# qiangbo1222/HierDiff

Hardware: AMD Instinct MI355X
Metric: sampled molecules/sec (1000 diffusion steps, B=256, N=30) (higher is better)
Workload: dtype f32

## Files before the change

### hierdiff_amd/build.py

```python
from __future__ import annotations

import os
import shutil
import subprocess
import sys

PKG = os.path.dirname(os.path.abspath(__file__))
CSRC = os.path.join(PKG, "csrc")
LIBDIR = os.path.join(PKG, "lib")
LIB = os.path.join(LIBDIR, "libhierdiff_hip.so")
SOURCES = [os.path.join(CSRC, "hierdiff_hip.hip")]
DEPS = SOURCES + [os.path.join(CSRC, f) for f in sorted(os.listdir(CSRC)) if f.endswith(".hpp")] + [
    os.path.join(os.path.dirname(PKG), "include", "hierdiff_hip.h")]


def _hipcc() -> str:
    for cand in (os.environ.get("HIPCC"), shutil.which("hipcc"), "/opt/rocm/bin/hipcc"):
        if cand and os.path.exists(cand):
            return cand
    raise RuntimeError("hipcc not found (set HIPCC)")


def needs_build() -> bool:
    if not os.path.exists(LIB):
        return True
    t = os.path.getmtime(LIB)
    return any(os.path.getmtime(d) > t for d in DEPS)


RESOURCES = os.path.join(LIBDIR, "kernel_resources.json")
KERNEL_FLAGS = ["--offload-arch=gfx950", "-O3", "-fno-slp-vectorize", "-std=c++17"]


def _parse_resource_remarks(text: str) -> dict:
    import re
    out, cur = {}, None
    for line in text.splitlines():
        m = re.search(r"remark: Function Name: (\S+)", line)
        if m:
            cur = out.setdefault(m.group(1), {})
            continue
        m = re.search(r"remark:\s+([A-Za-z][A-Za-z /\[\]]*?)(?: \[[^\]]*\])?: (\S+) \[-Rpass", line)
        if m and cur is not None:
            key = m.group(1).strip()
            try:
                cur[key] = int(m.group(2))
            except ValueError:
                cur[key] = m.group(2)
    return out


def _production(name: str) -> bool:
    import re
    m = re.match(r"_Z6k_edgeILi\d+ELb[01]ELi[03]ELi(\d+)EE", name)
    if m:
        return m.group(1) == "0"
    return True


def audit(resources: dict) -> list:
    bad = []
    for name, r in resources.items():
        if not name.startswith("_Z") or not _production(name):
            continue
        if r.get("ScratchSize", 0) or r.get("VGPRs Spill", 0):
            bad.append(f"{name}: scratch {r.get('ScratchSize')} B/lane, VGPR spills {r.get('VGPRs Spill')}")
    return bad


LIB_DEBUG = os.path.join(LIBDIR, "libhierdiff_hip_dbg.so")


def build(force: bool = False, save_temps: bool = False, verbose: bool = True, debug_kernels: bool = False) -> str:
    if debug_kernels:
        return _build_debug(verbose)
    if not force and not needs_build() and os.path.exists(RESOURCES):
        return LIB
    os.makedirs(LIBDIR, exist_ok=True)
    cmd = [_hipcc()] + KERNEL_FLAGS + ["-fPIC", "-shared",
           "-Wall", "-Wno-unused-function", "-Wno-unused-value", "-Wno-unused-result",
           "-Rpass-analysis=kernel-resource-usage", "-o", LIB + ".tmp"] + SOURCES
    if save_temps:
        tmpdir = os.path.join(PKG, "build")
        os.makedirs(tmpdir, exist_ok=True)
        cmd += ["-save-temps=obj"]
    if verbose:
        print(" ".join(cmd), flush=True)
    proc = subprocess.run(cmd, cwd=CSRC, stderr=subprocess.PIPE, text=True)
    other = [ln for ln in proc.stderr.splitlines() if "-Rpass-analysis=kernel-resource-usage" not in ln
             and not ln.startswith("In file included from")]
    if other and (verbose or proc.returncode):
        print("\n".join(other), file=sys.stderr, flush=True)
    if proc.returncode:
        raise subprocess.CalledProcessError(proc.returncode, cmd)
    resources = _parse_resource_remarks(proc.stderr)
    import json
    with open(RESOURCES, "w") as fh:
        json.dump(resources, fh, indent=1, sort_keys=True)
    bad = audit(resources)
    if bad:
        raise RuntimeError("register spills in production kernels (unsafe next to inline-asm loads):\n  " + "\n  ".join(bad))
    os.replace(LIB + ".tmp", LIB)
    return LIB


def _build_debug(verbose: bool = True) -> str:
    os.makedirs(LIBDIR, exist_ok=True)
    cmd = [_hipcc(), "-DHD_DEBUG_KERNELS"] + KERNEL_FLAGS + ["-fPIC",
           "-shared", "-Wno-unused-function", "-Wno-unused-value", "-Wno-unused-result", "-o", LIB_DEBUG] + SOURCES
    if verbose:
        print(" ".join(cmd), flush=True)
    subprocess.run(cmd, cwd=CSRC, check=True)
    return LIB_DEBUG


if __name__ == "__main__":
    print(build(force="--force" in sys.argv, save_temps="--save-temps" in sys.argv,
                debug_kernels="--debug-kernels" in sys.argv))
```

### hierdiff_amd/csrc/hierdiff_hip.hip

```cpp
#include "../../include/hierdiff_hip.h"
#include "kernels.hpp"

#include <algorithm>
#include <array>
#include <cmath>
#include <cstdio>
#include <cstring>
#include <cstdlib>
#include <string>
#include <mutex>
#include <vector>


static thread_local std::string g_err;

static int fail(int code, const std::string& msg) {
    g_err = msg;
    return code;
}

#define HIP_TRY(expr)                                                                        \
    do {                                                                                     \
        hipError_t _e = (expr);                                                              \
        if (_e != hipSuccess)                                                                \
// ... 1232 lines not shown
        case 1024: run(std::integral_constant<int, 1024>{}); return true;
        case 1025: run(std::integral_constant<int, 1025>{}); return true;
        default: return false;
    }
}
#else
extern "C" int hd_debug_edge_trace(hd_handle*, long long*, int) { return 0; }
#endif

static bool edge_runs_split(const hd_handle* h, int n_tiles, int mode) {
    return n_tiles > 0 && n_tiles <= (mode == 0 ? h->split_max_tiles + h->split_max_tiles / 3 : h->split_max_tiles);
}
static bool edge_runs_mixed(const hd_handle* h, int n_tiles, int mode) {
    const int per_round = 4 * h->n_cu;
    const int left = n_tiles - (n_tiles / per_round) * per_round;
    const bool pays = left > 0 && left * 10 <= (mode == 0 ? 29 : 10) * h->n_cu;
    return n_tiles > per_round && n_tiles < h->mix_max_tiles && (pays || h->mix_rounds >= 0);
}

template <int H>
static int launch_edge_h(hd_handle* h, bool coord, const EdgeArgs& a, hipStream_t s, int mode_override = -1) {
    const int lds = edge_lds_bytes<H>();
    const int prec = mode_override >= 0 ? mode_override : h->edge_mode;
    const dim3 grid(a.n_wg), block(256);
    if constexpr (H >= 128) {
        if (a.dscal) {
            if (a.pre2) {
                if (coord) hipLaunchKernelGGL((k_edge<H, true, 3, HD_EDGE_SAVE | HD_EDGE_UNSCALED>), grid, block, lds, s, a);
                else hipLaunchKernelGGL((k_edge<H, false, 3, HD_EDGE_SAVE | HD_EDGE_UNSCALED>), grid, block, lds, s, a);
            } else {
                if (coord) hipLaunchKernelGGL((k_edge<H, true, 3, HD_EDGE_UNSCALED>), grid, block, lds, s, a);
                else hipLaunchKernelGGL((k_edge<H, false, 3, HD_EDGE_UNSCALED>), grid, block, lds, s, a);
            }
            return HD_OK;
        }
    }
    if (a.pre2) {
        if (coord) hipLaunchKernelGGL((k_edge<H, true, 0, HD_EDGE_SAVE>), grid, block, lds, s, a);
        else hipLaunchKernelGGL((k_edge<H, false, 0, HD_EDGE_SAVE>), grid, block, lds, s, a);
        return HD_OK;
    }
#ifdef HD_DEBUG_KERNELS
    if constexpr (H == 256) {
        if (h->ablate && !coord && (prec == 3 ? launch_edge_ablated<3>(h, a, s) : launch_edge_ablated<0>(h, a, s))) return HD_OK;
    }
#endif
    if constexpr (H >= 128) {
        const int mode = prec;
        if (edge_runs_split(h, a.n_tiles, mode)) {
            const dim3 sgrid(a.n_tiles);
            if (mode == 0) {
                if (coord) hipLaunchKernelGGL((k_edge_split<H, true, 0>), sgrid, block, 0, s, a);
                else hipLaunchKernelGGL((k_edge_split<H, false, 0>), sgrid, block, 0, s, a);
            } else {
                if (coord) hipLaunchKernelGGL((k_edge_split<H, true, 3>), sgrid, block, 0, s, a);
                else hipLaunchKernelGGL((k_edge_split<H, false, 3>), sgrid, block, 0, s, a);
            }
            return HD_OK;
        }
    }
    if constexpr (H >= 128) {
        const int mode = prec;
        const int per_round = 4 * h->n_cu;
        int R = a.n_tiles / per_round;
        if (edge_runs_mixed(h, a.n_tiles, mode)) {
            if (h->mix_rounds >= 0) R = std::min(R, h->mix_rounds);
            EdgeArgs m = a;
            m.n_wg = R * h->n_cu;
            const dim3 mgrid(m.n_wg + (a.n_tiles - 4 * m.n_wg));
            const int ldsm = std::max(edge_lds_bytes<H>(), edge_split_lds_bytes<H>());
            if (mode == 0) {
                if (coord) hipLaunchKernelGGL((k_edge_mixed<H, true, 0>), mgrid, block, ldsm, s, m);
                else hipLaunchKernelGGL((k_edge_mixed<H, false, 0>), mgrid, block, ldsm, s, m);
            } else {
                if (coord) hipLaunchKernelGGL((k_edge_mixed<H, true, 3>), mgrid, block, ldsm, s, m);
                else hipLaunchKernelGGL((k_edge_mixed<H, false, 3>), mgrid, block, ldsm, s, m);
            }
            return HD_OK;
        }
    }
    if (prec == 3) {
        if (coord) hipLaunchKernelGGL((k_edge<H, true, 3>), grid, block, lds, s, a);
        else hipLaunchKernelGGL((k_edge<H, false, 3>), grid, block, lds, s, a);
    } else {
        if (coord) hipLaunchKernelGGL((k_edge<H, true, 0>), grid, block, lds, s, a);
        else hipLaunchKernelGGL((k_edge<H, false, 0>), grid, block, lds, s, a);
    }
    return HD_OK;
}

template <int H>
static int prepare_edge_h() {
    const int lds = edge_lds_bytes<H>();
    HIP_TRY(hipFuncSetAttribute((const void*)k_edge<H, true, 0>, hipFuncAttributeMaxDynamicSharedMemorySize, lds));
    HIP_TRY(hipFuncSetAttribute((const void*)k_edge<H, false, 0>, hipFuncAttributeMaxDynamicSharedMemorySize, lds));
    HIP_TRY(hipFuncSetAttribute((const void*)k_edge<H, true, 3>, hipFuncAttributeMaxDynamicSharedMemorySize, lds));
    HIP_TRY(hipFuncSetAttribute((const void*)k_edge<H, false, 3>, hipFuncAttributeMaxDynamicSharedMemorySize, lds));
    HIP_TRY(hipFuncSetAttribute((const void*)k_edge<H, true, 0, HD_EDGE_SAVE>, hipFuncAttributeMaxDynamicSharedMemorySize, lds));
    HIP_TRY(hipFuncSetAttribute((const void*)k_edge<H, false, 0, HD_EDGE_SAVE>, hipFuncAttributeMaxDynamicSharedMemorySize, lds));
    if constexpr (H >= 128) {
        HIP_TRY(hipFuncSetAttribute((const void*)k_edge<H, true, 3, HD_EDGE_SAVE | HD_EDGE_UNSCALED>, hipFuncAttributeMaxDynamicSharedMemorySize, lds));
        HIP_TRY(hipFuncSetAttribute((const void*)k_edge<H, false, 3, HD_EDGE_SAVE | HD_EDGE_UNSCALED>, hipFuncAttributeMaxDynamicSharedMemorySize, lds));
        HIP_TRY(hipFuncSetAttribute((const void*)k_edge<H, true, 3, HD_EDGE_UNSCALED>, hipFuncAttributeMaxDynamicSharedMemorySize, lds));
        HIP_TRY(hipFuncSetAttribute((const void*)k_edge<H, false, 3, HD_EDGE_UNSCALED>, hipFuncAttributeMaxDynamicSharedMemorySize, lds));
        const int m0 = std::max(edge_lds_bytes<H>(), edge_split_lds_bytes<H>());
        HIP_TRY(hipFuncSetAttribute((const void*)k_edge_mixed<H, true, 0>, hipFuncAttributeMaxDynamicSharedMemorySize, m0));
        HIP_TRY(hipFuncSetAttribute((const void*)k_edge_mixed<H, false, 0>, hipFuncAttributeMaxDynamicSharedMemorySize, m0));
        HIP_TRY(hipFuncSetAttribute((const void*)k_edge_mixed<H, true, 3>, hipFuncAttributeMaxDynamicSharedMemorySize, m0));
        HIP_TRY(hipFuncSetAttribute((const void*)k_edge_mixed<H, false, 3>, hipFuncAttributeMaxDynamicSharedMemorySize, m0));
    }
    return HD_OK;
}

static int prepare_kernels(hd_handle* h) {
    switch (h->H) {
        case 32: HD_TRY(prepare_node_h<32>()); HD_TRY(prepare_edge_bwd_h<32>()); return prepare_edge_h<32>();
        case 64: HD_TRY(prepare_node_h<64>()); HD_TRY(prepare_edge_bwd_h<64>()); return prepare_edge_h<64>();
        case 128: HD_TRY(prepare_node_h<128>()); HD_TRY(prepare_node_split_h<128>()); HD_TRY(prepare_edge_bwd_h<128>()); return prepare_edge_h<128>();
        default: HD_TRY(prepare_node_h<256>()); HD_TRY(prepare_node_split_h<256>()); HD_TRY(prepare_edge_bwd_h<256>()); return prepare_edge_h<256>();
    }
}

static int edge(hd_handle* h, bool coord, const EdgeArgs& a, hipStream_t s, int mode_override = -1) {
    if (a.n_wg == 0) return HD_OK;
    ProfScope ps(h, s, 0);
    switch (h->H) {
        case 32: return launch_edge_h<32>(h, coord, a, s, mode_override);
        case 64: return launch_edge_h<64>(h, coord, a, s, mode_override);
        case 128: return launch_edge_h<128>(h, coord, a, s, mode_override);
        default: return launch_edge_h<256>(h, coord, a, s, mode_override);
    }
}

static int forward_impl(hd_handle* h, hd_topology* t, const float* xh, const float* tt, int t_numel,
                        const float* context, int mol_shape, float* out, hipStream_t s) {
    const hd_config& c = h->cfg;
    const int H = h->H, M = t->M;
    const float* W = h->dw;
    h->prof_now = h->prof != 0 && (h->prof_fwd++ % h->prof_stride) == 0;
    if (M == 0) HIP_TRY(hipMemsetAsync(h->d_nanflag, 0, sizeof(int), s));
    if (M > 0) {
        {
            ProfScope ps(h, s, 2);
            InitArgs a;
            a.xh = xh; a.t = tt; a.ctx = context; a.node_of = t->node_of; a.nmask = t->nmask;
            a.embT = W + h->embT; a.emb_b = W + h->emb_b; a.h = t->hbuf; a.x0 = t->x0; a.xcur = t->xcur;
            a.nanflag = h->d_nanflag;
            a.zero_max = (h->node_mode == 3 && M < h->node_split_max_rows && h->edge_mode == 3) ? t->abmax : nullptr;
            a.M = M; a.N = t->N; a.D = h->D; a.F = h->F; a.C = c.context_node_nf; a.H = H;
            a.t_stride = (t_numel == 1) ? 0 : 1; a.cond_time = c.condition_time;
            const long long total = (long long)M * (H / 4);
            hipLaunchKernelGGL(k_node_init, dim3((unsigned)((total + 255) / 256)), dim3(256), 0, s, a);
        }
        const float range = c.coords_range / (float)c.n_layers;
        const int S = c.inv_sublayers;
        const float* ab_cur = t->AB;
        auto node_args = [&]() {
            NodeArgs a;
            std::memset(&a, 0, sizeof(a));
            a.h_in = t->hbuf; a.h_out = t->hbuf; a.part = t->part; a.pstart = t->pstart; a.nmask = t->nmask;
            a.norm = agg_norm(c, t); a.M = M;
            return a;
        };
        auto set_ab = [&](NodeArgs& a, int q, const LayerW& nw, float* dst) {
            a.ABimg[q] = W + nw.ab_img; a.ABbias[q] = W + nw.ab_bias; a.ABout[q] = dst;
            a.abinv[q] = h->node_mode == 3 ? 1.0f / nw.abs_ : 1.0f;
            a.ABmax[q] = (h->edge_mode == 3 && h->node_mode != 0) ? (dst == t->AB ? t->abmax : t->abmax2) : nullptr;
        };
        const bool fused = h->node_mode != 0 || M >= h->fuse_min_rows;
        auto r16_args = [&]() {
            R16Args g;
            std::memset(&g, 0, sizeof(g));
            g.A = t->hbuf; g.lda = H; g.K1 = H; g.K = H; g.M = M; g.n_img = 1; g.nmask = t->nmask; g.norm = agg_norm(c, t);
            return g;
        };
        auto ab_r16 = [&](int nab, const LayerW* const* nxt, float* const* dst) {
            R16Args g = r16_args();
            g.Nc = 2 * H; g.ldc = 2 * H; g.n_img = nab;
            for (int q = 0; q < nab; ++q) { g.Bimg[q] = W + nxt[q]->ab_gimg; g.bias[q] = W + nxt[q]->ab_bias; g.C[q] = dst[q]; }
            gemm_r16(h, EPI_BIAS, false, g, s);
        };
        const bool nsplit = h->node_mode == 3 && M < h->node_split_max_rows;
// ... 1311 lines not shown
```

### hierdiff_amd/csrc/k_edge.hpp

```cpp
#pragma once
#include "common.hpp"


#ifndef HD_F32_SILU
#define HD_F32_SILU silu_fast
#define HD_F32_SILU_IS_FAST 1
#endif

struct EdgeArgs {
    const float* AB;
    const float* wrd;
    const float* W2img;
    const float* b2;
    const float* wa;
    const int* ei;
    const int* ej;
    const uint8_t* eseg;
    const int* seg_part;
    const int* tile_nseg;
    const float* xcur;
    const float* x0;
    float* part;
    float ba;
    const float* ba_ptr;
    float norm_constant;
    float coords_range;
    int attention, use_tanh;
    int n_tiles, n_wg;
    long long* trace;
    float w2s_inv;
    float wrmax, wdmax;
    const float* abmax;
    const float* dscal;
    float* pre2;
};

constexpr int HD_EDGE_SAVE = 256;
constexpr int HD_EDGE_UNSCALED = 512;
constexpr float HD_NEG_LOG2E = -1.4426950408889634f;


struct AbMaxArgs { const float* AB; float* out; int M, H; };
__global__ void __launch_bounds__(256) k_ab_rowmax(AbMaxArgs a) {
    const int row = blockIdx.x * 4 + (threadIdx.x >> 6), lane = threadIdx.x & 63;
    if (row >= a.M) return;
    const float* r = a.AB + (size_t)row * 2 * a.H;
    float ma = 0.f, mb = 0.f;
    for (int k = 4 * lane; k < a.H; k += 256) {
        const f32x4 va = *reinterpret_cast<const f32x4*>(r + k), vb = *reinterpret_cast<const f32x4*>(r + a.H + k);
#pragma unroll
        for (int j = 0; j < 4; ++j) { ma = fmaxf(ma, fabsf(va[j])); mb = fmaxf(mb, fabsf(vb[j])); }
    }
#pragma unroll
    for (int o = 32; o > 0; o >>= 1) { ma = fmaxf(ma, __shfl_xor(ma, o)); mb = fmaxf(mb, __shfl_xor(mb, o)); }
    if (lane == 0) { a.out[2 * (size_t)row] = ma; a.out[2 * (size_t)row + 1] = mb; }
}


template <typename V, unsigned O0, unsigned O1, unsigned O2, unsigned O3>
HD_DEVINL void lds_read4(V (&f)[4], unsigned addr) {
    asm volatile("ds_read_b128 %0, %4 offset:%5\n\t"
                 "ds_read_b128 %1, %4 offset:%6\n\t"
                 "ds_read_b128 %2, %4 offset:%7\n\t"
                 "ds_read_b128 %3, %4 offset:%8"
                 : "=&v"(f[0]), "=&v"(f[1]), "=&v"(f[2]), "=&v"(f[3])
                 : "v"(addr), "i"(O0), "i"(O1), "i"(O2), "i"(O3));
}
template <typename V, unsigned O>
HD_DEVINL void lds_read1(V& f, unsigned addr) {
    asm volatile("ds_read_b128 %0, %1 offset:%2" : "=&v"(f) : "v"(addr), "i"(O));
}
template <int N, typename V>
HD_DEVINL void lds_wait4(V (&f)[4]) {
    asm volatile("s_waitcnt lgkmcnt(%4)" : "+v"(f[0]), "+v"(f[1]), "+v"(f[2]), "+v"(f[3]) : "i"(N));
}

HD_DEVINL float xhalf_sum(float x) {
    float lo = x, hi = x;
    asm("s_nop 1\n\tv_permlane32_swap_b32 %0, %1\n\ts_nop 1" : "+v"(lo), "+v"(hi));
    return lo + hi;
}
HD_DEVINL void xhalf_sum4(float (&x)[4]) {
    float lo[4], hi[4];
#pragma unroll
    for (int k = 0; k < 4; ++k) { lo[k] = x[k]; hi[k] = x[k]; }
    asm("s_nop 1\n\t"
        "v_permlane32_swap_b32 %0, %4\n\tv_permlane32_swap_b32 %1, %5\n\t"
        "v_permlane32_swap_b32 %2, %6\n\tv_permlane32_swap_b32 %3, %7\n\t"
        "s_nop 1"
        : "+v"(lo[0]), "+v"(lo[1]), "+v"(lo[2]), "+v"(lo[3]), "+v"(hi[0]), "+v"(hi[1]), "+v"(hi[2]), "+v"(hi[3]));
#pragma unroll
    for (int k = 0; k < 4; ++k) x[k] = lo[k] + hi[k];
}

HD_DEVINL void vm_load2(f32x4& va, f32x4& vb, const float* pa, const float* pb) {
    asm volatile("global_load_dwordx4 %0, %2, off\n\t"
                 "global_load_dwordx4 %1, %3, off"
                 : "=&v"(va), "=&v"(vb) : "v"(pa), "v"(pb));
}
template <int OFF>
HD_DEVINL void vm_load2o(f32x4& va, f32x4& vb, const float* pa, const float* pb) {
    static_assert(OFF >= 0 && OFF < 4096, "immediate offset out of range");
    asm volatile("global_load_dwordx4 %0, %2, off offset:%4\n\t"
                 "global_load_dwordx4 %1, %3, off offset:%4"
                 : "=&v"(va), "=&v"(vb) : "v"(pa), "v"(pb), "i"(OFF));
}
HD_DEVINL void vm_glds2(const float* ga, const float* gb, unsigned lds_a, unsigned lds_b) {
    unsigned keep;
    asm volatile("s_mov_b32 %0, m0\n\t"
                 "s_mov_b32 m0, %3\n\ts_nop 0\n\tglobal_load_lds_dwordx4 %1, off\n\t"
                 "s_mov_b32 m0, %4\n\ts_nop 0\n\tglobal_load_lds_dwordx4 %2, off\n\t"
                 "s_mov_b32 m0, %0"
                 : "=&s"(keep) : "v"(ga), "v"(gb), "s"(lds_a), "s"(lds_b));
}
template <int N, unsigned OA, unsigned OB>
HD_DEVINL void lds_read2_after_vm(f32x4& qa, f32x4& qb, unsigned addr) {
    asm volatile("s_waitcnt vmcnt(%3)\n\t"
                 "ds_read_b128 %0, %2 offset:%4\n\t"
                 "ds_read_b128 %1, %2 offset:%5"
                 : "=&v"(qa), "=&v"(qb) : "v"(addr), "i"(N), "i"(OA), "i"(OB));
}
HD_DEVINL void lds_ready2(f32x4& qa, f32x4& qb) { asm volatile("s_waitcnt lgkmcnt(0)" : "+v"(qa), "+v"(qb)); }
// ... 28 lines not shown
    constexpr int GL_PER_WAVE = (ABL & 128) ? CHF / (4 * 256) / 4 : CHF / (4 * 256);
    constexpr int LEVEL = edge_peel_level(H, PREC, ABL);
    static_assert(LEVEL >= 0 && LEVEL <= 2, "peel level");
    constexpr bool HAS_PEN = LEVEL >= 2, HAS_LAST = LEVEL >= 1;
    float* wbuf = smem;
    float* scratch = smem + 2 * CHF + 2 * H;

    const int tid = threadIdx.x, lane = tid & 63;
    const int wave = __builtin_amdgcn_readfirstlane(tid >> 6);
    const int hh = lane >> 5, n = lane & 31;
    float* my_scr = scratch + wave * 136;
    uint32_t* seg_s = reinterpret_cast<uint32_t*>(my_scr + 128);

    int wt;
    {
        const int xcd = bid & 7, slot = bid >> 3;
        const int q = nwt >> 3, r = nwt & 7;
        const int start = xcd < r ? xcd * (q + 1) : r * (q + 1) + (xcd - r) * q;
        const int len = q + (xcd < r ? 1 : 0);
        if (slot >= len) return;
        wt = start + slot;
    }
    long long ts0 = 0, ts1 = 0, ts2 = 0, ts3 = 0, ts4 = 0, ts5 = 0;
    if constexpr (ABL & 16) ts0 = __builtin_readcyclecounter();

    for (int k = tid; k < 2 * H; k += 256) wrd_s[k] = a.wrd[k];
    for (int k = tid; k < H; k += 256) { wrd_s[2 * H + k] = a.b2[k]; wrd_s[3 * H + k] = a.wa[k]; }
    auto issue_chunk = [&](int c, int buf) {
        const float* src = a.W2img + (size_t)c * CHF + wave * (GL_PER_WAVE * 256) + lane * 4;
        float* dst = wbuf + buf * CHF + wave * (GL_PER_WAVE * 256);
        static_for<0, GL_PER_WAVE>([&](auto U) {
            constexpr int u = decltype(U)::value;
            glds16o<(u & 3) * 1024>(src + (u >> 2) * 1024, dst + (u >> 2) * 1024);
        });
    };
    issue_chunk(0, 0);

    const int tile = wt * 4 + wave;
    const bool tile_ok = tile < a.n_tiles;
    int ni = 0, nj = 0;
    uint32_t segb = 255;
    if (tile_ok) {
        const int e = tile * 32 + n;
        ni = a.ei[e]; nj = a.ej[e]; segb = a.eseg[e];
    }

    int gc = 0;
    f32x4 xi = *reinterpret_cast<const f32x4*>(a.xcur + (size_t)ni * 4);
    f32x4 xj = *reinterpret_cast<const f32x4*>(a.xcur + (size_t)nj * 4);
    f32x4 yi = *reinterpret_cast<const f32x4*>(a.x0 + (size_t)ni * 4);
    f32x4 yj = *reinterpret_cast<const f32x4*>(a.x0 + (size_t)nj * 4);
    const float dx = xi[0] - xj[0], dy = xi[1] - xj[1], dz = xi[2] - xj[2];
    const float radial = dx * dx + dy * dy + dz * dz;
    if constexpr (COORD) {
        if (hh == 0) {
            const float inv = ((segb != 255) ? 1.0f : 0.0f) / (sqrtf(radial + 1e-8f) + a.norm_constant);
            float* tr = my_scr + 32;
            tr[n * 3 + 0] = dx * inv; tr[n * 3 + 1] = dy * inv; tr[n * 3 + 2] = dz * inv;
        }
    }
    const float ex = yi[0] - yj[0], ey = yi[1] - yj[1], ez = yi[2] - yj[2];
    const float d0 = ex * ex + ey * ey + ez * ez;
    const uint32_t segb_t = segb;
    float f16_inv = 1.0f;
    if constexpr (PREC == 3) {
        const float nodes = a.abmax[2 * (size_t)ni] + a.abmax[2 * (size_t)nj + 1] + HD_F16_FLOOR;
        const float wrmax = (ABL & HD_EDGE_UNSCALED) ? a.dscal[2] : a.wrmax, wdmax = (ABL & HD_EDGE_UNSCALED) ? a.dscal[3] : a.wdmax;
        const float bound = __builtin_fmaf(radial, wrmax, __builtin_fmaf(d0, wdmax, nodes));
        const uint32_t eb = (__builtin_bit_cast(uint32_t, bound) >> 23) & 0xffu;
        f16_inv = __builtin_bit_cast(float, (eb - 13u) << 23);
        if (hh == 0) my_scr[n] = f16_inv * ((ABL & HD_EDGE_UNSCALED) ? a.dscal[1] : a.w2s_inv);
    }
    const int pid_l = tile_ok ? a.seg_part[tile * 32 + n] : 0;
    const int nseg = tile_ok ? a.tile_nseg[tile] : 0;
    if (hh == 0) reinterpret_cast<uint8_t*>(seg_s)[n] = (uint8_t)segb_t;

    const float* Arow = a.AB + (size_t)ni * (2 * H) + (KC / 2) * hh;
    const float* Brow = a.AB + (size_t)nj * (2 * H) + H + (KC / 2) * hh;
    f32x4 pa[4], pb[4];
    auto rows_issue = [&](int u, int c) {
        if constexpr (ABL & 8) { pa[u] = f32x4{radial, d0, radial, d0}; pb[u] = pa[u]; }
        else vm_load2(pa[u], pb[u], Arow + KC * c + 4 * u, Brow + KC * c + 4 * u);
    };
    auto make_P = [&](int c, float (&P)[16]) {
#pragma unroll
        for (int u = 0; u < 4; ++u) {
            f32x4 wr4 = *reinterpret_cast<const f32x4*>(wrd_s + 32 * c + 16 * hh + 4 * u);
            f32x4 wd4 = *reinterpret_cast<const f32x4*>(wrd_s + H + 32 * c + 16 * hh + 4 * u);
#pragma unroll
            for (int j = 0; j < 4; ++j) {
                float pre = pa[u][j] + pb[u][j];
                pre = __builtin_fmaf(radial, wr4[j], pre);
                pre = __builtin_fmaf(d0, wd4[j], pre);
                P[4 * u + j] = HD_F32_SILU(pre);
            }
        }
    };
    auto make_quad = [&](f32x4 av, f32x4 bv, f32x4 wr4, f32x4 wd4, uint32_t (&hi)[2], uint32_t (&lo)[2]) {
        float pre[4], e[4];
#pragma unroll
        for (int j = 0; j < 4; ++j) pre[j] = av[j] + bv[j];
#pragma unroll
        for (int j = 0; j < 4; ++j) pre[j] = __builtin_fmaf(radial, wr4[j], pre[j]);
#pragma unroll
        for (int j = 0; j < 4; ++j) pre[j] = __builtin_fmaf(d0, wd4[j], pre[j]);
        if constexpr (ABL & 2) {
            f16_split2(av[0], av[1], hi[0], lo[0]);
            f16_split2(av[2], av[3], hi[1], lo[1]);
            return;
        }
#pragma unroll
        for (int j = 0; j < 4; ++j) e[j] = __builtin_amdgcn_exp2f((ABL & HD_EDGE_UNSCALED) ? pre[j] * HD_NEG_LOG2E : pre[j]);
#pragma unroll
        for (int j = 0; j < 4; ++j) e[j] = __builtin_fmaf(e[j], f16_inv, f16_inv);
#pragma unroll
        for (int j = 0; j < 4; ++j) e[j] = __builtin_amdgcn_rcpf(e[j]);
#pragma unroll
        for (int j = 0; j < 4; ++j) pre[j] *= e[j];
        f16_split2(pre[0], pre[1], hi[0], lo[0]);
        f16_split2(pre[2], pre[3], hi[1], lo[1]);
    };
    auto make_P_f16 = [&](int c, u32x4 (&ph)[2], u32x4 (&pl)[2]) {
#pragma unroll
        for (int u = 0; u < 4; ++u) {
            const f32x4 wr4 = *reinterpret_cast<const f32x4*>(wrd_s + 32 * c + 16 * hh + 4 * u);
            const f32x4 wd4 = *reinterpret_cast<const f32x4*>(wrd_s + H + 32 * c + 16 * hh + 4 * u);
            uint32_t hi[2], lo[2];
            make_quad(pa[u], pb[u], wr4, wd4, hi, lo);
            ph[u >> 1][2 * (u & 1)] = hi[0]; ph[u >> 1][2 * (u & 1) + 1] = hi[1];
            pl[u >> 1][2 * (u & 1)] = lo[0]; pl[u >> 1][2 * (u & 1) + 1] = lo[1];
        }
    };

    float Pc[16];
    u32x4 phc[2], plc[2];
    constexpr int NQ = KC / 8;
#pragma unroll
    for (int u = 0; u < NQ; ++u) rows_issue(u, 0);
    asm volatile("s_waitcnt vmcnt(0)" : "+v"(pa[0]), "+v"(pa[1]), "+v"(pa[2]), "+v"(pa[3]),
                                        "+v"(pb[0]), "+v"(pb[1]), "+v"(pb[2]), "+v"(pb[3]));
    __syncthreads();
    if constexpr (PREC == 0) make_P(0, Pc);
    else make_P_f16(0, phc, plc);
    if constexpr (NCH > 1 || !HAS_LAST) {
#pragma unroll
        for (int u = 0; u < NQ; ++u) rows_issue(u, NCH > 1 ? 1 : 0);
    }

    #ifdef HD_NO_PEEL
    constexpr bool PEEL = false;
#else
    constexpr bool PEEL = PREC == 3 && !(ABL & 2) && !(ABL & 1024);
#endif
    f32x16 acc[NCT];
    if constexpr (!PEEL) {
#pragma unroll
        for (int ct = 0; ct < NCT; ++ct) {
            const float b2v = PREC == 3 ? 0.0f : wrd_s[2 * H + 32 * ct + n];
#pragma unroll
            for (int r = 0; r < 16; ++r) acc[ct][r] = b2v;
        }
    }
    if constexpr (ABL & 16) ts1 = __builtin_readcyclecounter();
    constexpr int CH_MID = 0, CH_PEN = 1, CH_LAST = 2;
    auto chunk = [&](auto First, auto Kind, const int c) {
        constexpr bool FIRST = decltype(First)::value;
        constexpr int KIND = decltype(Kind)::value;
        const int buf = (ABL & 4) ? 0 : (gc & 1);
        if constexpr (!(ABL & 4) && !(ABL & 64)) {
            if constexpr (KIND == CH_LAST) {
                if constexpr (NCH > 1 && HAS_PEN) asm volatile("s_waitcnt vmcnt(0)\n\ts_barrier" ::: "memory");
                else if constexpr (NCH > 1) asm volatile("s_waitcnt vmcnt(8)\n\ts_barrier" ::: "memory");
            } else if constexpr (KIND == CH_PEN) {
                if constexpr (NCH > 2) asm volatile("s_waitcnt vmcnt(8)\n\ts_barrier" ::: "memory");
            } else {
                if (c > 0) asm volatile("s_waitcnt vmcnt(8)\n\ts_barrier" ::: "memory");
            }
            static_assert(HAS_LAST || KIND == CH_MID, "without a peeled last chunk every chunk runs the full body");
        }
        u32x4 phn[2], pln[2];
        const int cn1 = HAS_LAST ? c + 1 : (c + 1 < NCH ? c + 1 : NCH - 1);
        const int cn2 = HAS_PEN ? c + 2 : (c + 2 < NCH ? c + 2 : NCH - 1);
        const int cstream = HAS_LAST ? c + 1 : (c + 1 < NCH ? c + 1 : 0);
        auto rows_wait = [&](auto Q) {
            constexpr int q = decltype(Q)::value;
            static_assert(KIND != CH_LAST, "the last chunk waits for no rows");
            vm_wait2<(KIND == CH_MID ? 6 : 6 - 2 * q) + GL_PER_WAVE>(pa[q], pb[q]);
        };
        const float* Arow_n2 = Arow + KC * cn2;
        const float* Brow_n2 = Brow + KC * cn2;
        const float* wb = wbuf + buf * CHF;
        const unsigned wb_lds = (unsigned)(size_t)(__attribute__((address_space(3))) const void*)wb + lane * 16;
        if constexpr (PREC == 0) {
            constexpr int HC = NCT >= 4 ? 4 : NCT;
            constexpr int UPQ = NCT / HC;
            constexpr int NU = 4 * UPQ;
            f32x4 f0[4], f1[4];
            auto read_unit = [&](auto U, f32x4 (&f)[4]) {
                constexpr int u = decltype(U)::value, q = u / UPQ, c0 = (u % UPQ) * HC;
                lds_read4<f32x4, frag_off_f32(q * NCT + c0), frag_off_f32(q * NCT + c0 + (HC > 1 ? 1 : 0)),
                          frag_off_f32(q * NCT + c0 + (HC > 2 ? 2 : 0)), frag_off_f32(q * NCT + c0 + (HC > 3 ? 3 : 0))>(f, wb_lds);
            };
            read_unit(std::integral_constant<int, 0>{}, f0);
            if constexpr (KIND != CH_LAST && !(ABL & 4) && !(ABL & 32)) issue_chunk(cstream, buf ^ 1);
            static_for<0, NU>([&](auto Uc) {
                constexpr int u = decltype(Uc)::value, q = u / UPQ, c0 = (u % UPQ) * HC;
                f32x4(&cur)[4] = (u & 1) ? f1 : f0;
                f32x4(&nxt)[4] = (u & 1) ? f0 : f1;
                constexpr bool PRODUCE = KIND != CH_LAST && u % UPQ == UPQ - 1;
                lds_wait4<0>(cur);
                __builtin_amdgcn_sched_barrier(0);
                static_for<0, 4>([&](auto Ct) {
                    constexpr int ct = decltype(Ct)::value;
                    if constexpr (ct < HC) acc[c0 + ct] = __builtin_amdgcn_mfma_f32_32x32x2f32(Pc[4 * q], cur[ct][0], acc[c0 + ct], 0, 0, 0);
                    __builtin_amdgcn_sched_barrier(0);
                    if constexpr (u + 1 < NU) {
                        constexpr int qn = (u + 1) / UPQ, cn0 = ((u + 1) % UPQ) * HC;
                        lds_read1<f32x4, frag_off_f32(qn * NCT + cn0 + (ct < HC ? ct : 0))>(nxt[ct], wb_lds);
                    }
                    __builtin_amdgcn_sched_barrier(0);
                });
                f32x4 wr4, wd4;
                if constexpr (PRODUCE) {
                    wr4 = *reinterpret_cast<const f32x4*>(wrd_s + 32 * cn1 + 16 * hh + 4 * q);
                    wd4 = *reinterpret_cast<const f32x4*>(wrd_s + H + 32 * cn1 + 16 * hh + 4 * q);
                }
                __builtin_amdgcn_sched_barrier(0);
#pragma unroll
                for (int j = 1; j < 4; ++j)
#pragma unroll
                    for (int ct = 0; ct < HC; ++ct)
                        acc[c0 + ct] = __builtin_amdgcn_mfma_f32_32x32x2f32(Pc[4 * q + j], cur[ct][j], acc[c0 + ct], 0, 0, 0);
                __builtin_amdgcn_sched_barrier(0);
                if constexpr (PRODUCE) {
                    rows_wait(std::integral_constant<int, q>{});
#pragma unroll
                    for (int j = 0; j < 4; ++j) {
                        float pre = pa[q][j] + pb[q][j];
                        pre = __builtin_fmaf(radial, wr4[j], pre);
                        pre = __builtin_fmaf(d0, wd4[j], pre);
                        Pc[4 * q + j] = HD_F32_SILU(pre);
                    }
                    if constexpr (KIND == CH_MID) {
                        if constexpr (ABL & 8) { pa[q] = f32x4{radial, d0, radial, d0}; pb[q] = pa[q]; }
                        else vm_load2o<16 * q>(pa[q], pb[q], Arow_n2, Brow_n2);
                    }
                }
            });
        } else {
            constexpr int NG = NCT;
            const float* wr_n = wrd_s + 32 * cn1 + 16 * hh;
            const float* wd_n = wrd_s + H + 32 * cn1 + 16 * hh;
            f32x4 wrq[2], wdq[2];
            if constexpr (KIND != CH_LAST) {
                wrq[0] = *reinterpret_cast<const f32x4*>(wr_n);
                wdq[0] = *reinterpret_cast<const f32x4*>(wd_n);
            }
            f16x8 f0[4], f1[4];
            lds_read4<f16x8, frag_off_f16<NCT>(0, 0), frag_off_f16<NCT>(0, 1), frag_off_f16<NCT>(1, 0), frag_off_f16<NCT>(1, 1)>(f0, wb_lds);
            if constexpr (KIND != CH_LAST && !(ABL & 4) && !(ABL & 32)) issue_chunk(cstream, buf ^ 1);
            static_for<0, NG>([&](auto Gc) {
                constexpr int g = decltype(Gc)::value;
                f16x8(&cur)[4] = (g & 1) ? f1 : f0;
                f16x8(&nxt)[4] = (g & 1) ? f0 : f1;
                lds_wait4<0>(cur);
                if constexpr (g + 1 < NG) {
                    constexpr int u = 2 * (g + 1);
                    lds_read4<f16x8, frag_off_f16<NCT>(u, 0), frag_off_f16<NCT>(u, 1), frag_off_f16<NCT>(u + 1, 0),
                              frag_off_f16<NCT>(u + 1, 1)>(nxt, wb_lds);
                }
                __builtin_amdgcn_sched_barrier(0);
                constexpr int NGP = NG >= 2 ? NG / 2 : 1;
                constexpr int PPG = 8 / NGP;
                if constexpr (KIND != CH_LAST && g < NGP) {
                    static_for<0, PPG / 2>([&](auto V) {
                        constexpr int u = g * (PPG / 2) + decltype(V)::value;
                        rows_wait(std::integral_constant<int, u>{});
                        if constexpr (u + 1 < 4) {
                            wrq[(u + 1) & 1] = *reinterpret_cast<const f32x4*>(wr_n + 4 * (u + 1));
                            wdq[(u + 1) & 1] = *reinterpret_cast<const f32x4*>(wd_n + 4 * (u + 1));
                        }
                        uint32_t hi[2], lo[2];
                        make_quad(pa[u], pb[u], wrq[u & 1], wdq[u & 1], hi, lo);
                        phn[u >> 1][2 * (u & 1)] = hi[0]; phn[u >> 1][2 * (u & 1) + 1] = hi[1];
                        pln[u >> 1][2 * (u & 1)] = lo[0]; pln[u >> 1][2 * (u & 1) + 1] = lo[1];
                        if constexpr (KIND == CH_MID) {
                            if constexpr (ABL & 8) { pa[u] = f32x4{radial, d0, radial, d0}; pb[u] = pa[u]; }
                            else vm_load2o<16 * u>(pa[u], pb[u], Arow_n2, Brow_n2);
                        }
                    });
                }
                constexpr int u0 = 2 * g, u1 = 2 * g + 1;
                constexpr int s0 = u0 / NCT, c0 = u0 % NCT, s1 = u1 / NCT, c1 = u1 % NCT;
                const f16x8 A_h0 = __builtin_bit_cast(f16x8, phc[s0]), A_l0 = __builtin_bit_cast(f16x8, plc[s0]);
                const f16x8 A_h1 = __builtin_bit_cast(f16x8, phc[s1]), A_l1 = __builtin_bit_cast(f16x8, plc[s1]);
                if constexpr (ABL & 1024) {
                    asm volatile("" :: "v"(A_h0), "v"(A_l0), "v"(A_h1), "v"(A_l1), "v"(cur[0]), "v"(cur[1]), "v"(cur[2]), "v"(cur[3]));
                } else {
                if constexpr (FIRST && s0 == 0) acc[c0] = mma_f16(A_h0, cur[0], f32x16{});
                else acc[c0] = mma_f16(A_h0, cur[0], acc[c0]);
                if constexpr (FIRST && s1 == 0) acc[c1] = mma_f16(A_h1, cur[2], f32x16{});
                else acc[c1] = mma_f16(A_h1, cur[2], acc[c1]);
                acc[c0] = mma_f16(A_l0, cur[0], acc[c0]);
                acc[c1] = mma_f16(A_l1, cur[2], acc[c1]);
                acc[c0] = mma_f16(A_h0, cur[1], acc[c0]);
                acc[c1] = mma_f16(A_h1, cur[3], acc[c1]);
                }
                if constexpr (KIND != CH_LAST) {
#pragma unroll
                    for (int k = 0; k < 6; ++k) {
                        __builtin_amdgcn_sched_group_barrier(0x008, 1, 0);
                        __builtin_amdgcn_sched_group_barrier(0x002, 4, 0);
                    }
                }
                __builtin_amdgcn_sched_barrier(0);
            });
            if constexpr (KIND != CH_LAST) {
#pragma unroll
                for (int st = 0; st < 2; ++st) { phc[st] = phn[st]; plc[st] = pln[st]; }
            }
        }
    };
    using KMid = std::integral_constant<int, CH_MID>;
    using KPen = std::integral_constant<int, CH_PEN>;
    using KLast = std::integral_constant<int, CH_LAST>;
    if constexpr (!HAS_LAST) {
        if constexpr (PEEL) { chunk(std::true_type{}, KMid{}, 0); ++gc; }
#pragma unroll 1
        for (int c = PEEL ? 1 : 0; c < NCH; ++c, ++gc) chunk(std::false_type{}, KMid{}, c);
    } else if constexpr (NCH == 1) {
        chunk(std::bool_constant<PEEL>{}, KLast{}, 0);
    } else if constexpr (NCH == 2) {
        chunk(std::bool_constant<PEEL>{}, std::conditional_t<HAS_PEN, KPen, KMid>{}, 0); ++gc;
        chunk(std::false_type{}, KLast{}, 1);
    } else {
        if constexpr (PEEL) { chunk(std::true_type{}, KMid{}, 0); ++gc; }
#pragma unroll 1
        for (int c = PEEL ? 1 : 0; c < NCH - (HAS_PEN ? 2 : 1); ++c, ++gc) chunk(std::false_type{}, KMid{}, c);
        if constexpr (HAS_PEN) { chunk(std::false_type{}, KPen{}, NCH - 2); ++gc; }
        chunk(std::false_type{}, KLast{}, NCH - 1);
    }

    asm volatile("s_waitcnt vmcnt(0)" : "+v"(pa[0]), "+v"(pa[1]), "+v"(pa[2]), "+v"(pa[3]),
                                        "+v"(pb[0]), "+v"(pb[1]), "+v"(pb[2]), "+v"(pb[3]));
    if constexpr (ABL & 16) ts2 = __builtin_readcyclecounter();
    if constexpr (ABL & 1024) {
#pragma unroll
        for (int ct = 0; ct < NCT; ++ct)
#pragma unroll
            for (int r = 0; r < 16; ++r) asm volatile("" : "+v"(acc[ct][r]));
    }
    if constexpr (ABL & HD_EDGE_SAVE) {
        static_assert(PREC == 0 || (ABL & HD_EDGE_UNSCALED), "the saved pre-activations are those of the unscaled modes");
        if constexpr (PREC == 3) {
#pragma unroll
            for (int ct = 0; ct < NCT; ++ct) {
                const float b2v = wrd_s[2 * H + 32 * ct + n];
#pragma unroll
                for (int q = 0; q < 4; ++q) {
                    const f32x4 rs = *reinterpret_cast<const f32x4*>(my_scr + 8 * q + 4 * hh);
#pragma unroll
                    for (int j = 0; j < 4; ++j) acc[ct][4 * q + j] = __builtin_fmaf(acc[ct][4 * q + j], rs[j], b2v);
                }
            }
        }
        float* dst = a.pre2 + (size_t)tile * (32 * H) + lane * 4;
#pragma unroll
        for (int ct = 0; ct < NCT; ++ct)
#pragma unroll
            for (int q = 0; q < 4; ++q)
                *reinterpret_cast<f32x4*>(dst + (ct * 4 + q) * 256) = f32x4{acc[ct][4 * q], acc[ct][4 * q + 1], acc[ct][4 * q + 2], acc[ct][4 * q + 3]};
    }
    if (!tile_ok) return;
    if constexpr (ABL & 1) {
        float sacc = 0.f;
#pragma unroll
        for (int ct = 0; ct < NCT; ++ct)
#pragma unroll
            for (int r = 0; r < 16; ++r) sacc += acc[ct][r];
        if (sacc == 123.456f) a.part[lane] = sacc;
        return;
    }

    float dot[16];
#pragma unroll
    for (int r = 0; r < 16; ++r) dot[r] = 0.f;
    f32x4 rsc[4];
    if constexpr (PREC == 3) {
#pragma unroll
        for (int q = 0; q < 4; ++q) rsc[q] = *reinterpret_cast<const f32x4*>(my_scr + 8 * q + 4 * hh);
    }
#pragma unroll
    for (int ct = 0; ct < NCT; ++ct) {
        const float wav = wrd_s[3 * H + 32 * ct + n];
        if constexpr (PREC == 0) {
#ifdef HD_F32_SILU_IS_FAST
            float e[16];
#pragma unroll
            for (int r = 0; r < 16; ++r) e[r] = acc[ct][r] * -1.44269502162933349609375f;
            __builtin_amdgcn_sched_barrier(0);
#pragma unroll
            for (int r = 0; r < 16; ++r) e[r] = __builtin_amdgcn_exp2f(e[r]);
            __builtin_amdgcn_sched_barrier(0);
#pragma unroll
            for (int r = 0; r < 16; ++r) e[r] = 1.0f + e[r];
            __builtin_amdgcn_sched_barrier(0);
#pragma unroll
            for (int r = 0; r < 16; ++r) e[r] = __builtin_amdgcn_rcpf(e[r]);
            __builtin_amdgcn_sched_barrier(0);
#pragma unroll
            for (int r = 0; r < 16; ++r) acc[ct][r] *= e[r];
            __builtin_amdgcn_sched_barrier(0);
#pragma unroll
            for (int r = 0; r < 16; ++r) dot[r] = __builtin_fmaf(acc[ct][r], wav, dot[r]);
            __builtin_amdgcn_sched_barrier(0);
#else
#pragma unroll
            for (int r = 0; r < 16; ++r) {
                const float mv = HD_F32_SILU(acc[ct][r]);
                acc[ct][r] = mv;
                dot[r] = __builtin_fmaf(mv, wav, dot[r]);
            }
#endif
        } else {
            float e[16];
            if constexpr (!(ABL & HD_EDGE_SAVE)) {
                const float b2v = wrd_s[2 * H + 32 * ct + n];
#pragma unroll
                for (int r = 0; r < 16; ++r) acc[ct][r] = __builtin_fmaf(acc[ct][r], rsc[r >> 2][r & 3], b2v);
                __builtin_amdgcn_sched_barrier(0);
            }
#pragma unroll
            for (int r = 0; r < 16; ++r) e[r] = __builtin_amdgcn_exp2f((ABL & HD_EDGE_UNSCALED) ? acc[ct][r] * HD_NEG_LOG2E : acc[ct][r]);
            __builtin_amdgcn_sched_barrier(0);
#pragma unroll
            for (int r = 0; r < 16; ++r) e[r] = 1.0f + e[r];
            __builtin_amdgcn_sched_barrier(0);
#pragma unroll
            for (int r = 0; r < 16; ++r) e[r] = __builtin_amdgcn_rcpf(e[r]);
            __builtin_amdgcn_sched_barrier(0);
#pragma unroll
            for (int r = 0; r < 16; ++r) acc[ct][r] *= e[r];
            __builtin_amdgcn_sched_barrier(0);
#pragma unroll
            for (int r = 0; r < 16; ++r) dot[r] = __builtin_fmaf(acc[ct][r], wav, dot[r]);
            __builtin_amdgcn_sched_barrier(0);
        }
    }
    if constexpr (ABL & 16) ts3 = __builtin_readcyclecounter();
    float rowdot;
    {
        float v8[8], v4[4], v2[2];
        const bool b4 = n & 16, b3 = n & 8, b2_ = n & 4, b1 = n & 2;
#pragma unroll
        for (int k = 0; k < 8; ++k) {
            const float send = b4 ? dot[k] : dot[k + 8];
            const float keep = b4 ? dot[k + 8] : dot[k];
            v8[k] = keep + __shfl_xor(send, 16);
        }
#pragma unroll
        for (int k = 0; k < 4; ++k) {
            const float send = b3 ? v8[k] : v8[k + 4];
            const float keep = b3 ? v8[k + 4] : v8[k];
            v4[k] = keep + __shfl_xor(send, 8);
        }
#pragma unroll
        for (int k = 0; k < 2; ++k) {
            const float send = b2_ ? v4[k] : v4[k + 2];
            const float keep = b2_ ? v4[k + 2] : v4[k];
            v2[k] = keep + __shfl_xor(send, 4);
        }
        {
            const float send = b1 ? v2[0] : v2[1];
            const float keep = b1 ? v2[1] : v2[0];
            rowdot = keep + __shfl_xor(send, 2);
        }
        rowdot += __shfl_xor(rowdot, 1);
    }
    if constexpr (ABL & 16) ts4 = __builtin_readcyclecounter();
    const int my_slot = (n >> 1) & 15;

    if (!COORD) {
        uint32_t sw[4];
#pragma unroll
        for (int q = 0; q < 4; ++q) sw[q] = seg_s[2 * q + hh];
        float att_mine = 1.0f;
        if (a.attention) {
            const float ba = a.ba_ptr ? *a.ba_ptr : a.ba;
            if constexpr (PREC == 0) att_mine = sigmoid_f(rowdot + ba);
            else att_mine = __builtin_amdgcn_rcpf(1.0f + __builtin_amdgcn_exp2f((ABL & HD_EDGE_UNSCALED) ? (rowdot + ba) * HD_NEG_LOG2E : rowdot + ba));
        }
        float w[16];
        int sg[16];
#pragma unroll
        for (int r = 0; r < 16; ++r) {
            sg[r] = (sw[r >> 2] >> (8 * (r & 3))) & 255;
            const float att = __shfl(att_mine, (lane & 32) | (2 * r));
            w[r] = (sg[r] != 255) ? att : 0.0f;
        }
        if constexpr (ABL & 16) ts5 = __builtin_readcyclecounter();
        const bool tile_has_nan = __builtin_amdgcn_ballot_w64(rowdot != rowdot) != 0;
        for (int s = 0; s < nseg; ++s) {
            float ws[16];
#pragma unroll
            for (int r = 0; r < 16; ++r) ws[r] = (sg[r] == s) ? w[r] : 0.0f;
            float* dst = a.part + (size_t)__builtin_amdgcn_readlane(pid_l, s) * H + n;
            float sums[NCT];
            if (__builtin_expect(tile_has_nan, 0)) {
#pragma unroll
                for (int ct = 0; ct < NCT; ++ct) {
                    float sum = 0.f;
#pragma unroll
                    for (int r = 0; r < 16; ++r) sum = (sg[r] == s) ? __builtin_fmaf(ws[r], acc[ct][r], sum) : sum;
                    sums[ct] = sum;
                }
            } else {
#pragma unroll
                for (int ct = 0; ct < NCT; ++ct) {
                    float sum = 0.f;
#pragma unroll
                    for (int r = 0; r < 16; ++r) sum = __builtin_fmaf(ws[r], acc[ct][r], sum);
                    sums[ct] = sum;
                }
            }
            if constexpr (NCT % 4 == 0) {
#pragma unroll
                for (int c4 = 0; c4 < NCT; c4 += 4) {
                    float q4[4] = {sums[c4], sums[c4 + 1], sums[c4 + 2], sums[c4 + 3]};
                    xhalf_sum4(q4);
#pragma unroll
                    for (int k = 0; k < 4; ++k) sums[c4 + k] = q4[k];
                }
            } else {
#pragma unroll
                for (int ct = 0; ct < NCT; ++ct) sums[ct] = xhalf_sum(sums[ct]);
            }
            if (hh == 0) {
#pragma unroll
                for (int ct = 0; ct < NCT; ++ct) dst[32 * ct] = sums[ct];
            }
        }
    } else {
        if ((n & 1) == 0) my_scr[(my_slot & 3) + 8 * (my_slot >> 2) + 4 * hh] = rowdot;
        __builtin_amdgcn_wave_barrier();
        __builtin_amdgcn_fence(__ATOMIC_ACQ_REL, "wavefront");
        if (hh == 0) {
            float phi = my_scr[n];
            float sc = a.use_tanh ? tanhf(phi) * a.coords_range : phi;
            float* tr = my_scr + 32;
            tr[n * 3 + 0] *= sc;
            tr[n * 3 + 1] *= sc;
            tr[n * 3 + 2] *= sc;
        }
        __builtin_amdgcn_wave_barrier();
        __builtin_amdgcn_fence(__ATOMIC_ACQ_REL, "wavefront");
        if (lane < nseg) {
            const uint8_t* sb = reinterpret_cast<const uint8_t*>(seg_s);
            const float* tr = my_scr + 32;
            float sx = 0.f, sy = 0.f, sz = 0.f;
            for (int rr = 0; rr < 32; ++rr) {
                if (sb[rr] == lane) { sx += tr[rr * 3]; sy += tr[rr * 3 + 1]; sz += tr[rr * 3 + 2]; }
            }
            f32x4 o = {sx, sy, sz, 0.f};
            *reinterpret_cast<f32x4*>(a.part + (size_t)pid_l * 4) = o;
        }
        __builtin_amdgcn_wave_barrier();
        __builtin_amdgcn_fence(__ATOMIC_ACQ_REL, "wavefront");
    }
    if constexpr (ABL & 16) {
        if (lane == 0) {
            long long* t = a.trace + ((size_t)blockIdx.x * 4 + wave) * 8;
            const long long hw = __builtin_amdgcn_s_getreg((16 - 1) << 11 | 4) & 0xffff;
            const long long xcc = __builtin_amdgcn_s_getreg((4 - 1) << 11 | 20) & 0xf;
            t[0] = (ts0 & 0xffffffffffffll) | (hw << 48); t[1] = (ts1 & 0xffffffffffffll) | (xcc << 48);
            const long long m48 = 0xffffffffffffll;
            t[2] = ts2 & m48; t[3] = __builtin_readcyclecounter() & m48; t[4] = ts3 & m48; t[5] = ts4 & m48; t[6] = ts5 & m48; t[7] = nseg;
        }
    }
}

template <int H, bool COORD, int PREC, int ABL = 0>
__global__ __launch_bounds__(256, 2) void k_edge(EdgeArgs a) {
    extern __shared__ __attribute__((aligned(16))) float smem[];
    __shared__ __attribute__((aligned(16))) float wrd_s[4 * H];
    edge_tile_body<H, COORD, PREC, ABL>(a, smem, wrd_s, blockIdx.x, a.n_wg);
}
```

Baseline: 48.69.

## Add packed-f32 SiLU edge variant and skip empty segment groups in scatter

```diff
diff --git a/hierdiff_amd/build.py b/hierdiff_amd/build.py
--- a/hierdiff_amd/build.py
+++ b/hierdiff_amd/build.py
@@ -58,13 +58,20 @@
     return True
 
 
+def _packed_edge(name: str) -> bool:
+    import re
+    return re.match(r"_Z6k_edgeILi\d+ELb[01]ELi0ELi2048EE", name) is not None
+
+
 def audit(resources: dict) -> list:
     bad = []
     for name, r in resources.items():
-        if not name.startswith("_Z") or not _production(name):
+        if not name.startswith("_Z") or not (_production(name) or _packed_edge(name)):
             continue
         if r.get("ScratchSize", 0) or r.get("VGPRs Spill", 0):
             bad.append(f"{name}: scratch {r.get('ScratchSize')} B/lane, VGPR spills {r.get('VGPRs Spill')}")
+        elif _packed_edge(name) and r.get("VGPRs", 0) + r.get("AGPRs", 0) > 256:
+            bad.append(f"{name}: {r.get('VGPRs')} VGPRs + {r.get('AGPRs')} AGPRs, more than 256")
     return bad
 
 
diff --git a/hierdiff_amd/csrc/hierdiff_hip.hip b/hierdiff_amd/csrc/hierdiff_hip.hip
--- a/hierdiff_amd/csrc/hierdiff_hip.hip
+++ b/hierdiff_amd/csrc/hierdiff_hip.hip
@@ -1338,6 +1338,9 @@
     if (prec == 3) {
         if (coord) hipLaunchKernelGGL((k_edge<H, true, 3>), grid, block, lds, s, a);
         else hipLaunchKernelGGL((k_edge<H, false, 3>), grid, block, lds, s, a);
+    } else if constexpr (edge_packed_width(H)) {
+        if (coord) hipLaunchKernelGGL((k_edge<H, true, 0, HD_EDGE_PACKED>), grid, block, lds, s, a);
+        else hipLaunchKernelGGL((k_edge<H, false, 0, HD_EDGE_PACKED>), grid, block, lds, s, a);
     } else {
         if (coord) hipLaunchKernelGGL((k_edge<H, true, 0>), grid, block, lds, s, a);
         else hipLaunchKernelGGL((k_edge<H, false, 0>), grid, block, lds, s, a);
@@ -1354,6 +1357,10 @@
     HIP_TRY(hipFuncSetAttribute((const void*)k_edge<H, false, 3>, hipFuncAttributeMaxDynamicSharedMemorySize, lds));
     HIP_TRY(hipFuncSetAttribute((const void*)k_edge<H, true, 0, HD_EDGE_SAVE>, hipFuncAttributeMaxDynamicSharedMemorySize, lds));
     HIP_TRY(hipFuncSetAttribute((const void*)k_edge<H, false, 0, HD_EDGE_SAVE>, hipFuncAttributeMaxDynamicSharedMemorySize, lds));
+    if constexpr (edge_packed_width(H)) {
+        HIP_TRY(hipFuncSetAttribute((const void*)k_edge<H, true, 0, HD_EDGE_PACKED>, hipFuncAttributeMaxDynamicSharedMemorySize, lds));
+        HIP_TRY(hipFuncSetAttribute((const void*)k_edge<H, false, 0, HD_EDGE_PACKED>, hipFuncAttributeMaxDynamicSharedMemorySize, lds));
+    }
     if constexpr (H >= 128) {
         HIP_TRY(hipFuncSetAttribute((const void*)k_edge<H, true, 3, HD_EDGE_SAVE | HD_EDGE_UNSCALED>, hipFuncAttributeMaxDynamicSharedMemorySize, lds));
         HIP_TRY(hipFuncSetAttribute((const void*)k_edge<H, false, 3, HD_EDGE_SAVE | HD_EDGE_UNSCALED>, hipFuncAttributeMaxDynamicSharedMemorySize, lds));
diff --git a/hierdiff_amd/csrc/k_edge.hpp b/hierdiff_amd/csrc/k_edge.hpp
--- a/hierdiff_amd/csrc/k_edge.hpp
+++ b/hierdiff_amd/csrc/k_edge.hpp
@@ -38,6 +38,17 @@
 constexpr int HD_EDGE_SAVE = 256;
 constexpr int HD_EDGE_UNSCALED = 512;
 constexpr float HD_NEG_LOG2E = -1.4426950408889634f;
+constexpr int HD_EDGE_PACKED = 2048;
+constexpr bool edge_packed_width(int H) {
+#ifdef HD_EDGE_NO_PACKED
+    return false;
+#else
+    return H >= 256;
+#endif
+}
+HD_DEVINL f32x2 pk_fma(f32x2 a, f32x2 b, f32x2 c) { return __builtin_elementwise_fma(a, b, c); }
+HD_DEVINL f32x2 pk2(float lo, float hi) { return f32x2{lo, hi}; }
+HD_DEVINL f32x2 pk_splat(float v) { return f32x2{v, v}; }
 
 
 struct AbMaxArgs { const float* AB; float* out; int M, H; };
@@ -232,11 +243,35 @@
         if constexpr (ABL & 8) { pa[u] = f32x4{radial, d0, radial, d0}; pb[u] = pa[u]; }
         else vm_load2(pa[u], pb[u], Arow + KC * c + 4 * u, Brow + KC * c + 4 * u);
     };
+    constexpr bool PACKED = PREC == 0 && (ABL & HD_EDGE_PACKED) != 0;
+#ifndef HD_F32_SILU_IS_FAST
+    static_assert(!PACKED, "the packed form is silu_fast written out");
+#endif
+    auto make_quad_pk = [&](const f32x4 av, const f32x4 bv, const f32x4 wr4, const f32x4 wd4, float (&P)[16], const int at) {
+        f32x2 pre[2], e[2];
+#pragma unroll
+        for (int p = 0; p < 2; ++p) pre[p] = pk2(av[2 * p], av[2 * p + 1]) + pk2(bv[2 * p], bv[2 * p + 1]);
+#pragma unroll
+        for (int p = 0; p < 2; ++p) pre[p] = pk_fma(pk_splat(radial), pk2(wr4[2 * p], wr4[2 * p + 1]), pre[p]);
+#pragma unroll
+        for (int p = 0; p < 2; ++p) pre[p] = pk_fma(pk_splat(d0), pk2(wd4[2 * p], wd4[2 * p + 1]), pre[p]);
+#pragma unroll
+        for (int p = 0; p < 2; ++p) e[p] = pre[p] * pk_splat(-1.44269502162933349609375f);
+#pragma unroll
+        for (int p = 0; p < 2; ++p) e[p] = pk2(__builtin_amdgcn_exp2f(e[p][0]), __builtin_amdgcn_exp2f(e[p][1]));
+#pragma unroll
+        for (int p = 0; p < 2; ++p) e[p] = pk_splat(1.0f) + e[p];
+#pragma unroll
+        for (int p = 0; p < 2; ++p) e[p] = pk2(__builtin_amdgcn_rcpf(e[p][0]), __builtin_amdgcn_rcpf(e[p][1]));
+#pragma unroll
+        for (int p = 0; p < 2; ++p) { pre[p] = pre[p] * e[p]; P[at + 2 * p] = pre[p][0]; P[at + 2 * p + 1] = pre[p][1]; }
+    };
     auto make_P = [&](int c, float (&P)[16]) {
 #pragma unroll
         for (int u = 0; u < 4; ++u) {
             f32x4 wr4 = *reinterpret_cast<const f32x4*>(wrd_s + 32 * c + 16 * hh + 4 * u);
             f32x4 wd4 = *reinterpret_cast<const f32x4*>(wrd_s + H + 32 * c + 16 * hh + 4 * u);
+            if constexpr (PACKED) { make_quad_pk(pa[u], pb[u], wr4, wd4, P, 4 * u); continue; }
 #pragma unroll
             for (int j = 0; j < 4; ++j) {
                 float pre = pa[u][j] + pb[u][j];
@@ -383,13 +418,17 @@
                         acc[c0 + ct] = __builtin_amdgcn_mfma_f32_32x32x2f32(Pc[4 * q + j], cur[ct][j], acc[c0 + ct], 0, 0, 0);
                 __builtin_amdgcn_sched_barrier(0);
                 if constexpr (PRODUCE) {
+                    if constexpr (PACKED) asm volatile("" :: "v"(acc[c0 + HC - 1]));
                     rows_wait(std::integral_constant<int, q>{});
-#pragma unroll
-                    for (int j = 0; j < 4; ++j) {
-                        float pre = pa[q][j] + pb[q][j];
-                        pre = __builtin_fmaf(radial, wr4[j], pre);
-                        pre = __builtin_fmaf(d0, wd4[j], pre);
-                        Pc[4 * q + j] = HD_F32_SILU(pre);
+                    if constexpr (PACKED) make_quad_pk(pa[q], pb[q], wr4, wd4, Pc, 4 * q);
+                    else {
+#pragma unroll
+                        for (int j = 0; j < 4; ++j) {
+                            float pre = pa[q][j] + pb[q][j];
+                            pre = __builtin_fmaf(radial, wr4[j], pre);
+                            pre = __builtin_fmaf(d0, wd4[j], pre);
+                            Pc[4 * q + j] = HD_F32_SILU(pre);
+                        }
                     }
                     if constexpr (KIND == CH_MID) {
                         if constexpr (ABL & 8) { pa[q] = f32x4{radial, d0, radial, d0}; pb[q] = pa[q]; }
@@ -545,6 +584,31 @@
         const float wav = wrd_s[3 * H + 32 * ct + n];
         if constexpr (PREC == 0) {
 #ifdef HD_F32_SILU_IS_FAST
+            if constexpr (PACKED) {
+                f32x2 x2[8], e2[8];
+#pragma unroll
+                for (int p = 0; p < 8; ++p) { x2[p] = pk2(acc[ct][2 * p], acc[ct][2 * p + 1]); e2[p] = x2[p] * pk_splat(-1.44269502162933349609375f); }
+                __builtin_amdgcn_sched_barrier(0);
+#pragma unroll
+                for (int p = 0; p < 8; ++p) e2[p] = pk2(__builtin_amdgcn_exp2f(e2[p][0]), __builtin_amdgcn_exp2f(e2[p][1]));
+                __builtin_amdgcn_sched_barrier(0);
+#pragma unroll
+                for (int p = 0; p < 8; ++p) e2[p] = pk_splat(1.0f) + e2[p];
+                __builtin_amdgcn_sched_barrier(0);
+#pragma unroll
+                for (int p = 0; p < 8; ++p) e2[p] = pk2(__builtin_amdgcn_rcpf(e2[p][0]), __builtin_amdgcn_rcpf(e2[p][1]));
+                __builtin_amdgcn_sched_barrier(0);
+#pragma unroll
+                for (int p = 0; p < 8; ++p) { x2[p] = x2[p] * e2[p]; acc[ct][2 * p] = x2[p][0]; acc[ct][2 * p + 1] = x2[p][1]; }
+                __builtin_amdgcn_sched_barrier(0);
+#pragma unroll
+                for (int p = 0; p < 8; ++p) {
+                    const f32x2 d2 = pk_fma(x2[p], pk_splat(wav), pk2(dot[2 * p], dot[2 * p + 1]));
+                    dot[2 * p] = d2[0]; dot[2 * p + 1] = d2[1];
+                }
+                __builtin_amdgcn_sched_barrier(0);
+                continue;
+            }
             float e[16];
 #pragma unroll
             for (int r = 0; r < 16; ++r) e[r] = acc[ct][r] * -1.44269502162933349609375f;
@@ -650,27 +714,34 @@
         }
         if constexpr (ABL & 16) ts5 = __builtin_readcyclecounter();
         const bool tile_has_nan = __builtin_amdgcn_ballot_w64(rowdot != rowdot) != 0;
-        for (int s = 0; s < nseg; ++s) {
-            float ws[16];
-#pragma unroll
-            for (int r = 0; r < 16; ++r) ws[r] = (sg[r] == s) ? w[r] : 0.0f;
+        uint32_t sq[8];
+#pragma unroll
+        for (int k = 0; k < 8; ++k) sq[k] = __builtin_amdgcn_readfirstlane(seg_s[k]);
+        const int nseg_u = __builtin_amdgcn_readfirstlane(nseg);
+        for (int s = 0; s < nseg_u; ++s) {
             float* dst = a.part + (size_t)__builtin_amdgcn_readlane(pid_l, s) * H + n;
+            const uint32_t s4 = (uint32_t)s * 0x01010101u;
             float sums[NCT];
-            if (__builtin_expect(tile_has_nan, 0)) {
-#pragma unroll
-                for (int ct = 0; ct < NCT; ++ct) {
-                    float sum = 0.f;
-#pragma unroll
-                    for (int r = 0; r < 16; ++r) sum = (sg[r] == s) ? __builtin_fmaf(ws[r], acc[ct][r], sum) : sum;
-                    sums[ct] = sum;
-                }
-            } else {
-#pragma unroll
-                for (int ct = 0; ct < NCT; ++ct) {
-                    float sum = 0.f;
-#pragma unroll
-                    for (int r = 0; r < 16; ++r) sum = __builtin_fmaf(ws[r], acc[ct][r], sum);
-                    sums[ct] = sum;
+#pragma unroll
+            for (int ct = 0; ct < NCT; ++ct) sums[ct] = 0.f;
+#pragma unroll
+            for (int q = 0; q < 4; ++q) {
+                const uint32_t x0 = sq[2 * q] ^ s4, x1 = sq[2 * q + 1] ^ s4;
+                if (((((x0 - 0x01010101u) & ~x0) | ((x1 - 0x01010101u) & ~x1)) & 0x80808080u) == 0) continue;
+                float ws[4];
+#pragma unroll
+                for (int j = 0; j < 4; ++j) ws[j] = (sg[4 * q + j] == s) ? w[4 * q + j] : 0.0f;
+                if (__builtin_expect(tile_has_nan, 0)) {
+#pragma unroll
+                    for (int ct = 0; ct < NCT; ++ct)
+#pragma unroll
+                        for (int j = 0; j < 4; ++j)
+                            sums[ct] = (sg[4 * q + j] == s) ? __builtin_fmaf(ws[j], acc[ct][4 * q + j], sums[ct]) : sums[ct];
+                } else {
+#pragma unroll
+                    for (int ct = 0; ct < NCT; ++ct)
+#pragma unroll
+                        for (int j = 0; j < 4; ++j) sums[ct] = __builtin_fmaf(ws[j], acc[ct][4 * q + j], sums[ct]);
                 }
             }
             if constexpr (NCT % 4 == 0) {
```

After: 49.34 (median of 6 runs). 1.01x the previous value.
